# vressegu/sdeflow-light

Measured on AMD Instinct MI355X. Metric: score-matching train steps/sec (+ reverse-SDE sample steps/sec), higher is better.
Workload: dtype f32

## Files before the change

### sdeflow_light_amd/csrc/conv_kernels.hip

```cpp
#include "common.h"
#include <algorithm>
#include <type_traits>
#include <stdlib.h>

#define CONV_MAX_SRC 2

struct ConvGeom {
  int N, Hi, Wi, Ho, Wo;
  int KH, KW, strideH, padH, strideW, padW;
  int mode;
  int ups;
};

struct ConvArgs {
  ConvGeom g;
  const float* src[CONV_MAX_SRC];
  int C[CONV_MAX_SRC];
  int koff[CONV_MAX_SRC];
  int nsrc;
  const float* Wp;
  int Cout, CoutP, Ktot;
  const float* bias;
  const float* samp_bias;
  int n_bias, n_samp;
// ... 597 lines not shown
          if (dy > py || dx > px) continue;
          const int kh = py ? (dy ? 0 : 2) : 1, kw = px ? (dx ? 0 : 2) : 1;
          const float* wp = wl + (size_t)(kh * 3 + kw) * tap_stride + c0 + 16 * grp;
          f32x4 a[2];
#pragma unroll
          for (int c = 0; c < 2; ++c) a[c] = *reinterpret_cast<const f32x4*>(wp + c * co_stride);
#pragma unroll
          for (int r = 0; r < 4; ++r)
#pragma unroll
            for (int c = 0; c < 2; ++c)
#pragma unroll
              for (int pt = 0; pt < 2; ++pt) acc[cls][c][pt] = mfma16(a[c][r], b[pt][r], acc[cls][c][pt]);
        }
      }
    }
  }
  asm volatile("s_nop 15\n\ts_nop 7" ::: "memory");
  __builtin_amdgcn_sched_barrier(0);
#pragma unroll
  for (int c = 0; c < 2; ++c) {
    const int co = co0 + 16 * c + 4 * q;
    const f32x4 add = conv_addend(A, n, co, true);
    f32x4 cs = {0.f, 0.f, 0.f, 0.f}, css = cs;
#pragma unroll
    for (int pt = 0; pt < 2; ++pt) {
      const int yy = y0 + 2 * w + pt, xx = x0 + il;
      if (yy >= g.Hi || xx >= g.Wi) continue;
#pragma unroll
      for (int cls = 0; cls < 4; ++cls) {
        const size_t m = ((size_t)n * g.Ho + 2 * yy + (cls >> 1)) * g.Wo + 2 * xx + (cls & 1);
        conv_store_quad(A, A.out + m * A.Cout + co, acc[cls][c][pt] + add, true, co, cs, css);
      }
    }
  }
}

#define C1_LP 36
template <int PT, int KG, int EXTRA>
__global__ void __launch_bounds__(256) k_conv1x1(ConvArgs A, int P , long Mtot, int ct_per) {
  constexpr bool LDS_OUT = PT == 4;
  __shared__ __attribute__((aligned(16))) float c1_lds[4][LDS_OUT ? 16 * PT * C1_LP : 4];
  const int tid = threadIdx.x, w = tid >> 6, lane = tid & 63, il = lane & 15, q = lane >> 4;
  const long m0 = ((long)blockIdx.x * 4 + w) * (16 * PT);
  if (m0 >= Mtot) return;
  float* wl = c1_lds[w];
  const int n = __builtin_amdgcn_readfirstlane((int)(m0 / P));
  const int g0 = A.C[0] >> 4;
  const int ctot = A.C[0] + (A.nsrc > 1 ? A.C[1] : 0);
  f32x4 b[PT][KG];
#pragma unroll
  for (int pt = 0; pt < PT; ++pt) {
    const long m = m0 + 16 * pt + il;
#pragma unroll
    for (int g = 0; g < KG; ++g) {
      const bool second = g >= g0;
      const int c = (second ? 16 * (g - g0) : 16 * g) + 4 * q;
      const int C = second ? A.C[1] : A.C[0];
      b[pt][g] = *reinterpret_cast<const f32x4*>((second ? A.src[1] : A.src[0]) + (size_t)m * C + c);
    }
  }
  if (A.in_scale) {
#pragma unroll
    for (int g = 0; g < KG; ++g) {
      const bool second = g >= g0;
      const size_t o = (size_t)n * ctot + (second ? A.C[0] + 16 * (g - g0) : 16 * g) + 4 * q;
      const f32x4 ga = *reinterpret_cast<const f32x4*>(A.in_scale + o), gb = *reinterpret_cast<const f32x4*>(A.in_shift + o);
#pragma unroll
      for (int pt = 0; pt < PT; ++pt) {
        f32x4 v = b[pt][g] * ga + gb;
        if (A.in_act == 1) {
#pragma unroll
          for (int r = 0; r < 4; ++r) v[r] = v[r] * __builtin_amdgcn_rcpf(1.0f + __expf(-v[r]));
        }
        b[pt][g] = v;
      }
    }
  }
  const int ct0 = blockIdx.y * ct_per, ntile = min(A.Cout >> 4, ct0 + ct_per);
  const float* wrow = A.Wp + (size_t)il * A.Ktot + 4 * q;
  const size_t tile_stride = (size_t)16 * A.Ktot;
  constexpr int D = (KG % 4 == 0) ? 4 : 2;
  static_assert(KG % D == 0 && D <= KG, "ring slots must line up from one tile to the next");
  f32x4 an[D];
#pragma unroll
  for (int d = 0; d < D; ++d) an[d] = *reinterpret_cast<const f32x4*>(wrow + (size_t)ct0 * tile_stride + 16 * d);
  const bool has_b = A.bias && n < A.n_bias, has_s = A.samp_bias && n < A.n_samp;
  const float fb = has_b ? 1.f : 0.f, fs = has_s ? 1.f : 0.f;
  const float* bp = has_b ? A.bias + 4 * q : A.Wp;
  const float* sp = has_s ? A.samp_bias + (size_t)n * A.Cout + 4 * q : A.Wp;
  const int bstep = has_b ? 16 : 0, sstep = has_s ? 16 : 0;
  f32x4 add_n = *reinterpret_cast<const f32x4*>(bp + (size_t)ct0 * bstep) * fb + *reinterpret_cast<const f32x4*>(sp + (size_t)ct0 * sstep) * fs;
  const float* ex = EXTRA ? (A.residual ? A.residual : A.out) : nullptr;
  const size_t orow = (size_t)(m0 + il) * A.Cout + 4 * q;
  const size_t ptstep = (size_t)16 * A.Cout;
  f32x4 ex_n[EXTRA ? PT : 1];
  if (EXTRA) {
#pragma unroll
    for (int pt = 0; pt < PT; ++pt) ex_n[pt] = *reinterpret_cast<const f32x4*>(ex + orow + pt * ptstep + 16 * ct0);
  }
  for (int ct = ct0; ct < ntile; ++ct) {
    const int ctn = min(ct + 1, ntile - 1);
    f32x4 acc[PT];
#pragma unroll
    for (int pt = 0; pt < PT; ++pt) acc[pt] = f32x4{0, 0, 0, 0};
    const f32x4 add = add_n;
    f32x4 exv[EXTRA ? PT : 1];
    if (EXTRA) {
#pragma unroll
      for (int pt = 0; pt < PT; ++pt) exv[pt] = ex_n[pt];
    }
#pragma unroll
    for (int g = 0; g < KG; ++g) {
      const f32x4 a = an[g % D];
      const int ng = (g + D < KG) ? g + D : g + D - KG, nct = (g + D < KG) ? ct : ctn;
      an[g % D] = *reinterpret_cast<const f32x4*>(wrow + (size_t)nct * tile_stride + 16 * ng);
      if (g == 0) {
        add_n = *reinterpret_cast<const f32x4*>(bp + (size_t)ctn * bstep) * fb + *reinterpret_cast<const f32x4*>(sp + (size_t)ctn * sstep) * fs;
        if (EXTRA) {
#pragma unroll
          for (int pt = 0; pt < PT; ++pt) ex_n[pt] = *reinterpret_cast<const f32x4*>(ex + orow + pt * ptstep + 16 * ctn);
        }
      }
      __builtin_amdgcn_sched_barrier(0);
#pragma unroll
      for (int r = 0; r < 4; ++r)
#pragma unroll
        for (int pt = 0; pt < PT; ++pt) acc[pt] = mfma16(a[r], b[pt][g][r], acc[pt]);
    }
    f32x4 cs = {0.f, 0.f, 0.f, 0.f}, css = {0.f, 0.f, 0.f, 0.f};
    const int half = (ct - ct0) & 1;
    const bool paired = LDS_OUT && (half == 1 || ct + 1 < ntile);
#pragma unroll
    for (int pt = 0; pt < PT; ++pt) {
      f32x4 v = acc[pt] + add;
      if (EXTRA) v += exv[pt];
      if (paired) *reinterpret_cast<f32x4*>(wl + (16 * pt + il) * C1_LP + 16 * half + 4 * q) = v;
      else *reinterpret_cast<f32x4*>(A.out + orow + pt * ptstep + 16 * ct) = v;
      cs += v; css += v * v;
    }
    if (LDS_OUT && half == 1) {
      const size_t obase = (size_t)m0 * A.Cout + 16 * (ct - 1) + 4 * (lane & 7);
#pragma unroll
      for (int j = 0; j < 2 * PT; ++j) {
        const int px = 8 * j + (lane >> 3);
        const f32x4 v = *reinterpret_cast<const f32x4*>(wl + px * C1_LP + 4 * (lane & 7));
        *reinterpret_cast<f32x4*>(A.out + obase + (size_t)px * A.Cout) = v;
        if (j & 1) __builtin_amdgcn_sched_barrier(0);
      }
    }
    if (A.cstat) cstat_store(A, n, (int)((m0 % P) / (16 * PT)), 16 * ct + 4 * q, cs, css, il);
  }
}

constexpr int H18_HW = 18, H18_ITEMS = H18_HW * H18_HW * (CT_KC / 4), H18_NST = (H18_ITEMS + 255) / 256;
__device__ __forceinline__ void halo18_load(const ConvArgs& A, const ConvGeom& g, const float* src, int C, int up, int c0, size_t aff0, int n, int y0, int x0,
                                            int tid, f32x4 (&st)[H18_NST], unsigned& valid, f32x4& ga, f32x4& gb) {
  const float* base = src + (size_t)n * g.Hi * g.Wi * C;
  const int cq = c0 + 4 * (tid & 7);
  ga = f32x4{1.f, 1.f, 1.f, 1.f}; gb = f32x4{0.f, 0.f, 0.f, 0.f};
  if (A.in_scale && cq < C) {
    const size_t o = aff0 + cq;
    ga = *reinterpret_cast<const f32x4*>(A.in_scale + o);
    gb = *reinterpret_cast<const f32x4*>(A.in_shift + o);
  }
  valid = 0;
#pragma unroll
  for (int k = 0; k < H18_NST; ++k) {
    const int idx = tid + 256 * k;
    f32x4 v = {0, 0, 0, 0};
    if (idx < H18_ITEMS) {
      const int hp = idx >> 3, hy = hp / H18_HW, hx = hp - hy * H18_HW;
      const int iy = y0 + hy - 1, ix = x0 + hx - 1;
      const int c = c0 + 4 * (idx & 7);
      if (iy >= 0 && iy < (g.Hi << up) && ix >= 0 && ix < (g.Wi << up) && c < C) {
        v = *reinterpret_cast<const f32x4*>(base + ((size_t)(iy >> up) * g.Wi + (ix >> up)) * C + c);
        valid |= 1u << k;
      }
    }
    st[k] = v;
  }
}
__device__ __forceinline__ void halo18_store(const ConvArgs& A, float* buf, int tid, f32x4 (&st)[H18_NST], unsigned valid, f32x4 ga, f32x4 gb) {
  if (A.in_scale) {
#pragma unroll
    for (int k = 0; k < H18_NST; ++k) {
      if ((valid >> k) & 1u) {
        f32x4 v = st[k] * ga + gb;
        if (A.in_act == 1) {
#pragma unroll
          for (int r = 0; r < 4; ++r) v[r] = v[r] * __builtin_amdgcn_rcpf(1.0f + __expf(-v[r]));
        }
        st[k] = v;
      }
    }
  }
#pragma unroll
  for (int k = 0; k < H18_NST; ++k) {
    const int idx = tid + 256 * k;
    if (idx < H18_ITEMS) *reinterpret_cast<f32x4*>(buf + (idx >> 3) * CT_P + 4 * (idx & 7)) = st[k];
  }
}

__device__ __forceinline__ float wave64_sum_to_last(float v) {
  v = row16_sum(v);
  v += __builtin_bit_cast(float, __builtin_amdgcn_update_dpp(0, __builtin_bit_cast(int, v), 0x142, 0xA, 0xF, false));
  v += __builtin_bit_cast(float, __builtin_amdgcn_update_dpp(0, __builtin_bit_cast(int, v), 0x143, 0xC, 0xF, false));
  return v;
}

template <int CO>
__global__ void __launch_bounds__(256) k_conv3x3_cin_small(ConvArgs A, long Mtot) {
  const ConvGeom g = A.g;
  const int P = g.Ho * g.Wo, Cin = A.C[0];
  const long m = (long)blockIdx.x * 256 + threadIdx.x;
  const bool live = m < Mtot;
  const long mm = live ? m : Mtot - 1;
  const int n = (int)(mm / P), r = (int)(mm - (long)n * P), y = r / g.Wo, x = r - y * g.Wo;
  const float* src = A.src[0] + (size_t)n * g.Hi * g.Wi * Cin;
  float acc[CO];
#pragma unroll
  for (int co = 0; co < CO; ++co) acc[co] = 0.f;
#pragma unroll
  for (int tap = 0; tap < 9; ++tap) {
    const int iy = y + tap / 3 - 1, ix = x + tap % 3 - 1;
    const bool ok = iy >= 0 && iy < g.Hi && ix >= 0 && ix < g.Wi;
    const float* px = src + ((size_t)(ok ? iy : 0) * g.Wi + (ok ? ix : 0)) * Cin;
    const float* wt = A.Wp + (size_t)(g.mode ? 8 - tap : tap) * A.CoutP * A.Ktot;
    for (int c = 0; c < Cin; ++c) {
      const float xv = ok ? px[c] : 0.f;
#pragma unroll
      for (int co = 0; co < CO; ++co) acc[co] = __builtin_fmaf(xv, wt[(size_t)co * A.Ktot + c], acc[co]);
    }
  }
  const bool primal = n < A.n_bias && A.bias;
  float* op = A.out + (size_t)mm * CO;
#pragma unroll
  for (int c4 = 0; c4 < CO / 4; ++c4) {
    f32x4 v = {acc[4 * c4], acc[4 * c4 + 1], acc[4 * c4 + 2], acc[4 * c4 + 3]};
    if (primal) v += *reinterpret_cast<const f32x4*>(A.bias + 4 * c4);
    if (A.samp_bias && n < A.n_samp) v += *reinterpret_cast<const f32x4*>(A.samp_bias + (size_t)n * CO + 4 * c4);
    if (live) {
      if (A.accumulate) v += *reinterpret_cast<const f32x4*>(op + 4 * c4);
      if (A.residual) v += *reinterpret_cast<const f32x4*>(A.residual + (size_t)mm * CO + 4 * c4);
      *reinterpret_cast<f32x4*>(op + 4 * c4) = v;
    } else {
      v = f32x4{0.f, 0.f, 0.f, 0.f};
    }
#pragma unroll
    for (int k = 0; k < 4; ++k) acc[4 * c4 + k] = v[k];
  }
  if (A.cstat) {
    const int lane = threadIdx.x & 63;
    float* cp = A.cstat + (((size_t)n * A.cs_S + (r >> 6)) * 2) * CO;
#pragma unroll
    for (int co = 0; co < CO; ++co) {
      const float s = wave64_sum_to_last(acc[co]), ss = wave64_sum_to_last(acc[co] * acc[co]);
      if (lane == 63 && live) { cp[co] = s; cp[CO + co] = ss; }
    }
  }
}

template <int CO>
__global__ void __launch_bounds__(256) k_conv3x3_cout_small(ConvArgs A, int tiles_x, int tiles_y) {
  extern __shared__ __attribute__((aligned(16))) float cs_lds[];
  const ConvGeom g = A.g;
  const int tid = threadIdx.x;
  constexpr int HW = H18_HW;
  int n, y0, x0;
  tile_origin<16, 16>(blockIdx.x, tiles_x, tiles_y, n, y0, x0);
  f32x4 st[H18_NST], ga, gb;
  unsigned valid;
  halo18_load(A, g, A.src[0], 32, 0, 0, (size_t)n * 32, n, y0, x0, tid, st, valid, ga, gb);
  halo18_store(A, cs_lds, tid, st, valid, ga, gb);
  __syncthreads();
  const int py = tid >> 4, px = tid & 15;
  float acc[CO];
#pragma unroll
  for (int co = 0; co < CO; ++co) acc[co] = 0.f;
#pragma unroll
  for (int tap = 0; tap < 9; ++tap) {
    const float* xp = cs_lds + ((py + tap / 3) * HW + px + tap % 3) * CT_P;
    const float* wt = A.Wp + (size_t)tap * A.CoutP * A.Ktot;
#pragma unroll
    for (int q4 = 0; q4 < 8; ++q4) {
      const f32x4 xv = *reinterpret_cast<const f32x4*>(xp + 4 * q4);
#pragma unroll
      for (int co = 0; co < CO; ++co) {
        const float* w = wt + (size_t)co * A.Ktot + 4 * q4;
        acc[co] = __builtin_fmaf(xv[0], w[0], acc[co]); acc[co] = __builtin_fmaf(xv[1], w[1], acc[co]);
        acc[co] = __builtin_fmaf(xv[2], w[2], acc[co]); acc[co] = __builtin_fmaf(xv[3], w[3], acc[co]);
      }
    }
#pragma unroll
    for (int co = 0; co < CO; ++co) asm volatile("" : "+v"(acc[co]));
  }
  const int oy = y0 + py, ox = x0 + px;
  if (oy < g.Ho && ox < g.Wo) {
    const size_t m = ((size_t)n * g.Ho + oy) * g.Wo + ox;
    float* op = A.out + m * CO;
#pragma unroll
    for (int co = 0; co < CO; ++co) {
      float v = acc[co];
      if (n < A.n_bias && A.bias) v += A.bias[co];
      if (A.samp_bias && n < A.n_samp) v += A.samp_bias[(size_t)n * CO + co];
      if (A.accumulate) v += op[co];
      if (A.residual) v += A.residual[m * CO + co];
// ... 1410 lines not shown
    if (dual) zt = *reinterpret_cast<const f32x4*>(z + half + 4 * i);
    f32x4 hp, ht;
#pragma unroll
    for (int k = 0; k < 4; ++k) {
      float a0, a1, a2;
      if (ACT == 0) gelu012(zp[k], a0, a1, a2); else silu012(zp[k], a0, a1, a2);
      hp[k] = a0; ht[k] = a1 * zt[k];
    }
    *reinterpret_cast<f32x4*>(h + 4 * i) = hp;
    if (dual) *reinterpret_cast<f32x4*>(h + half + 4 * i) = ht;
  }
}
template <int ACT>
__global__ void k_act_dual_bwd(const float* __restrict__ z, float* __restrict__ g, int64_t half) {
  const int64_t nq = half >> 2;
  for (int64_t i = blockIdx.x * (int64_t)blockDim.x + threadIdx.x; i < nq; i += (int64_t)gridDim.x * blockDim.x) {
    const f32x4 zp = *reinterpret_cast<const f32x4*>(z + 4 * i), zt = *reinterpret_cast<const f32x4*>(z + half + 4 * i);
    f32x4 gp = *reinterpret_cast<const f32x4*>(g + 4 * i), gt = *reinterpret_cast<const f32x4*>(g + half + 4 * i);
#pragma unroll
    for (int k = 0; k < 4; ++k) {
      float a0, a1, a2;
      if (ACT == 0) gelu012(zp[k], a0, a1, a2); else silu012(zp[k], a0, a1, a2);
      const float np = gp[k] * a1 + gt[k] * (a2 * zt[k]);
      gt[k] = gt[k] * a1;
      gp[k] = np;
    }
    *reinterpret_cast<f32x4*>(g + 4 * i) = gp;
    *reinterpret_cast<f32x4*>(g + half + 4 * i) = gt;
  }
}

__device__ __forceinline__ void slot_reduce_block(long blk, const float* __restrict__ part, int nslots, long stride, long n_elem,
                                                  float* __restrict__ out, int C, int Ktot, int koff, int accumulate,
                                                  int rowsP, int rows, long n_elem2, float* __restrict__ out2) {
  __shared__ float red[8][32];
  const int el = threadIdx.x & 31, sl = threadIdx.x >> 5;
  const long nb1 = (n_elem + 31) / 32;
  if (blk >= nb1) {
    const long e2 = (blk - nb1) * 32 + el;
    const bool ok2 = e2 < n_elem2;
    float t2 = 0.f;
    if (ok2)
      for (int s = sl; s < nslots; s += 8) t2 += part[(size_t)s * stride + n_elem + e2];
    red[sl][el] = t2;
    __syncthreads();
    if (sl == 0 && ok2) {
      float r = red[0][el];
#pragma unroll
      for (int k = 1; k < 8; ++k) r += red[k][el];
      out2[e2] = accumulate ? out2[e2] + r : r;
    }
    return;
  }
  const long e = blk * 32 + el;
  const bool ok = e < n_elem && (rowsP == 0 || (int)((e / C) % rowsP) < rows);
  float t = 0.f;
  if (ok)
    for (int s = sl; s < nslots; s += 8) t += part[(size_t)s * stride + e];
  red[sl][el] = t;
  __syncthreads();
  if (sl == 0 && ok) {
    float r = red[0][el];
#pragma unroll
    for (int k = 1; k < 8; ++k) r += red[k][el];
    const long o = Ktot > 0 ? (e / C) * Ktot + koff + (e % C) : e;
    out[o] = accumulate ? out[o] + r : r;
  }
}
__global__ void __launch_bounds__(256) k_slot_reduce(const float* __restrict__ part, int nslots, long stride, long n_elem,
                                                      float* __restrict__ out, int C, int Ktot, int koff, int accumulate,
                                                      int rowsP, int rows, long n_elem2, float* __restrict__ out2) {
  slot_reduce_block((long)blockIdx.x, part, nslots, stride, n_elem, out, C, Ktot, koff, accumulate, rowsP, rows, n_elem2, out2);
}
__global__ void __launch_bounds__(256) k_slot_reduce_batched(const msgm_reduce_job_t* __restrict__ jobs, int n_jobs) {
  int lo = 0, hi = n_jobs - 1;
  const long blk = blockIdx.x;
  while (lo < hi) {
    const int mid = (lo + hi + 1) >> 1;
    if (jobs[mid].block_begin <= blk) lo = mid; else hi = mid - 1;
  }
  const msgm_reduce_job_t J = jobs[lo];
  slot_reduce_block(blk - J.block_begin, J.part, J.nslots, (long)J.stride, (long)J.n_elem, J.out, J.C, J.Ktot, J.koff, J.accumulate,
                    J.rowsP, J.rows, (long)J.n_elem2, J.out2);
}

__global__ void __launch_bounds__(256) k_colsum(const float* __restrict__ x, float* __restrict__ S, int P, int C, int chunk) {
  __shared__ float red[256];
  const int n = blockIdx.x;
  const float* xn = x + (size_t)n * P * C;
  const int p0 = blockIdx.y * chunk, p1 = min(p0 + chunk, P);
  for (int cb = 0; cb < C; cb += 256) {
    const int lanes_c = min(C - cb, 256);
    const int rows = 256 / lanes_c;
    const int c = threadIdx.x % lanes_c, pr = threadIdx.x / lanes_c;
    float s = 0.f;
    if (pr < rows)
      for (int p = p0 + pr; p < p1; p += rows) s += xn[(size_t)p * C + cb + c];
    red[threadIdx.x] = (pr < rows) ? s : 0.f;
    __syncthreads();
    if (pr == 0) {
      float t = 0.f;
      for (int r = 0; r < rows; ++r) t += red[r * lanes_c + c];
      S[((size_t)blockIdx.y * gridDim.x + n) * C + cb + c] = t;
    }
    __syncthreads();
  }
}

__global__ void k_add_row(float* __restrict__ x, const float* __restrict__ E, int N, int P, int C, int pos, float sgn) {
  const int64_t tot = (int64_t)N * C;
  for (int64_t e = blockIdx.x * (int64_t)blockDim.x + threadIdx.x; e < tot; e += (int64_t)gridDim.x * blockDim.x) {
    const int n = (int)(e / C), c = (int)(e - (int64_t)n * C);
    x[((size_t)n * P + pos) * C + c] += sgn * E[e];
  }
}

__global__ void k_gather_row(const float* __restrict__ x, float* __restrict__ out, int N, int P, int C, int pos) {
  const int64_t tot = (int64_t)N * C;
  for (int64_t e = blockIdx.x * (int64_t)blockDim.x + threadIdx.x; e < tot; e += (int64_t)gridDim.x * blockDim.x) {
    const int n = (int)(e / C), c = (int)(e - (int64_t)n * C);
    out[e] = x[((size_t)n * P + pos) * C + c];
  }
}

static int check_geom(const msgm_conv_geom_t* g) {
  if (!g || g->N <= 0 || g->Hi <= 0 || g->Wi <= 0 || g->Ho <= 0 || g->Wo <= 0 || g->KH <= 0 || g->KW <= 0 ||
      g->strideH <= 0 || g->padH < 0 || g->strideW <= 0 || g->padW < 0 || (g->mode != 0 && g->mode != 1) ||
      (g->ups != 0 && g->ups != 1))
    return MSGM_E_BADARG;
  if ((int64_t)g->N * g->Ho * g->Wo >= (1ll << 31) || (int64_t)g->N * g->Hi * g->Wi >= (1ll << 31)) return MSGM_E_UNSUPPORTED;
  return MSGM_OK;
}
static ConvGeom to_geom(const msgm_conv_geom_t* g) {
  return ConvGeom{g->N, g->Hi, g->Wi, g->Ho, g->Wo, g->KH, g->KW, g->strideH, g->padH, g->strideW, g->padW, g->mode, g->ups};
}

static bool conv_same(const msgm_conv_geom_t* g) {
  const int ups_sh = g->ups ? 1 : 0;
  return g->strideH == 1 && g->strideW == 1 && (g->Hi << ups_sh) == g->Ho && (g->Wi << ups_sh) == g->Wo &&
         (g->KH & 1) && (g->KW & 1) && g->KH <= 3 && g->KW <= 3 && g->padH == (g->KH - 1) / 2 && g->padW == (g->KW - 1) / 2;
}

static int conv_n_cu() {
  static const int n_cu = [] { int d = 0, n = 256; (void)hipGetDevice(&d); (void)hipDeviceGetAttribute(&n, hipDeviceAttributeMultiprocessorCount, d); return n > 0 ? n : 256; }();
  return n_cu;
}
template <auto K, int BYTES = 160 * 1024>
static void conv_raise_lds_limit() {
  static const int once = [] {
    (void)hipFuncSetAttribute(reinterpret_cast<const void*>(K), hipFuncAttributeMaxDynamicSharedMemorySize, BYTES);
    return 0;
  }();
  (void)once;
}

extern "C" {

static bool conv_tile_eligible(const msgm_conv_geom_t* geom, int32_t C0, bool has1, int32_t C1, int32_t CoutP) {
  const bool fast = (C0 % 16 == 0) && (!has1 || C1 % 16 == 0);
  return conv_same(geom) && (!geom->ups || geom->mode == 0) && fast && CoutP % 32 == 0 && (int64_t)geom->Ho * geom->Wo >= 64 &&
         (geom->Ho > 1 ? geom->KH == geom->KW : geom->KH == 1);
}

static bool conv_wino_eligible(const msgm_conv_geom_t* geom, int32_t C0, int32_t C1, int32_t CoutP, int cmul) {
  return geom->mode == 0 && geom->KH == 3 && geom->KW == 3 && conv_same(geom) && geom->Ho % 16 == 0 && geom->Wo % 16 == 0 &&
         C0 % cmul == 0 && C1 % cmul == 0 && CoutP % 32 == 0;
}

int msgm_conv_wino_supported(const msgm_conv_geom_t* geom, int32_t C0, int32_t C1, int32_t CoutP) {
  if (check_geom(geom)) return 0;
  return conv_wino_eligible(geom, C0, C1, CoutP, 16) ? 1 : 0;
}

static int conv_args(ConvArgs* A, const msgm_conv_geom_t* geom, const float* src0, int32_t C0, const float* src1, int32_t C1,
                     const void* W, int32_t Cout, int32_t CoutP, int32_t Ktot, const float* bias, const float* samp_bias,
                     int32_t n_bias, int32_t n_samp, float* out, int32_t accumulate, const msgm_conv_fuse_t* fuse,
                     bool padded_k) {
  int rc = check_geom(geom);
  if (rc) return rc;
  if (fuse && ((fuse->in_scale == nullptr) != (fuse->in_shift == nullptr) || (fuse->in_act != 0 && fuse->in_act != 1)))
    return MSGM_E_BADARG;
  if (!src0 || !W || !out || C0 <= 0 || Cout <= 0 || (src1 && C1 <= 0)) return MSGM_E_BADARG;
  const int k0 = padded_k ? ((C0 + 15) / 16) * 16 : C0, k1 = !src1 ? 0 : padded_k ? ((C1 + 15) / 16) * 16 : C1;
  if (Ktot != k0 + k1 || CoutP % 16 || CoutP < Cout) return MSGM_E_BADARG;
  *A = ConvArgs{};
  A->g = to_geom(geom);
  A->src[0] = src0; A->C[0] = C0; A->koff[0] = 0;
  A->src[1] = src1; A->C[1] = src1 ? C1 : 0; A->koff[1] = k0;
  A->nsrc = src1 ? 2 : 1;
  A->Wp = static_cast<const float*>(W); A->Cout = Cout; A->CoutP = CoutP; A->Ktot = Ktot;
  A->bias = bias; A->samp_bias = samp_bias; A->n_bias = n_bias; A->n_samp = n_samp; A->out = out; A->accumulate = accumulate;
  if (fuse) {
    A->residual = fuse->residual; A->in_scale = fuse->in_scale; A->in_shift = fuse->in_shift; A->in_act = fuse->in_act;
    for (int i = 0; i < 16; ++i) A->tapmask_in[i] = fuse->tapmask_in[i];
    for (int i = 0; i < 8; ++i) A->tapmask_out[i] = fuse->tapmask_out[i];
    A->cstat = fuse->chanstats;
  }
  return MSGM_OK;
}
static bool conv_has_masks(const ConvArgs& A) {
  unsigned m = 0;
  for (int i = 0; i < 16; ++i) m |= A.tapmask_in[i];
  for (int i = 0; i < 8; ++i) m |= A.tapmask_out[i];
  return m != 0;
}

int msgm_wino_pack_weights_batched(const msgm_pack_job_t* jobs, int32_t n_jobs, msgm_stream_t stream) {
  if (!jobs || n_jobs <= 0) return MSGM_E_BADARG;
  hipLaunchKernelGGL(k_wino_pack_batched, dim3(8, (unsigned)n_jobs), dim3(256), 0, S(stream), jobs);
  return msgm_check_launch();
}

static bool tile16_chanstats(ConvArgs& A) {
  if (!A.cstat) return true;
  A.cs_S = (A.g.Wo / 16) * (A.g.Ho / 16) * 4;
  return A.Cout % 4 == 0;
}

int msgm_conv_forward_wino(const msgm_conv_geom_t* geom, const float* src0, int32_t C0, const float* src1, int32_t C1,
                           const float* WpW, int32_t Cout, int32_t CoutP, int32_t Ktot, const float* bias,
                           const float* samp_bias, int32_t n_bias, int32_t n_samp, float* out, int32_t accumulate,
                           const msgm_conv_fuse_t* fuse, msgm_stream_t stream) {
  ConvArgs A;
  int rc = conv_args(&A, geom, src0, C0, src1, C1, WpW, Cout, CoutP, Ktot, bias, samp_bias, n_bias, n_samp, out, accumulate,
                     fuse, true);
  if (rc) return rc;
  if (!conv_wino_eligible(geom, C0, A.C[1], CoutP, 16) || !tile16_chanstats(A)) return MSGM_E_UNSUPPORTED;
  const int tiles_x = geom->Wo / 16, tiles_y = geom->Ho / 16;
  const int n_tiles = tiles_x * tiles_y * geom->N, gy = CoutP / 32;
  if (!A.in_scale) {
    const int64_t lim = (int64_t)1 << 31;
    if ((int64_t)geom->Hi * geom->Wi * std::max(C0, A.C[1]) * 4 >= lim || (int64_t)16 * CoutP * Ktot * 4 >= lim) return MSGM_E_UNSUPPORTED;
    conv_raise_lds_limit<&k_conv_wino_pipe, WP_LDS_BYTES>();
    const int items_per_xcd = gy * ((n_tiles + 7) / 8);
    const int wg_per_xcd = std::min(items_per_xcd, std::max(1, 2 * conv_n_cu() / 8));
    hipLaunchKernelGGL(k_conv_wino_pipe, dim3((unsigned)(8 * wg_per_xcd)), dim3(256), WP_LDS_BYTES, S(stream), A, tiles_x, tiles_y, n_tiles, gy);
    return msgm_check_launch();
  }
  const size_t lds = (size_t)18 * 18 * CT_P * sizeof(float);
  dim3 grid((unsigned)(8 * gy * ((n_tiles + 7) / 8)));
  constexpr int p32_min = 1024;
  if (!src1 && Ktot == 32 && CoutP == 32 && n_tiles >= p32_min) {
    conv_raise_lds_limit<&k_conv_wino_p32>();
    const size_t lds32 = ((size_t)2 * 16 * 2 * 256 + 2 * 18 * 18 * CT_P) * sizeof(float);
    hipLaunchKernelGGL(k_conv_wino_p32, dim3((unsigned)conv_n_cu()), dim3(256), lds32, S(stream), A, tiles_x, tiles_y, n_tiles);
    return msgm_check_launch();
  }
  if (Ktot < 64) {
    hipLaunchKernelGGL((k_conv_wino<2, false>), grid, dim3(256), lds, S(stream), A, tiles_x, tiles_y, n_tiles, gy);
    return msgm_check_launch();
  }
  conv_raise_lds_limit<&k_conv_wino<2, true>>();
  hipLaunchKernelGGL((k_conv_wino<2, true>), grid, dim3(256), lds + 2 * 4096 * sizeof(float), S(stream), A, tiles_x, tiles_y, n_tiles, gy);
  return msgm_check_launch();
}

__global__ void __launch_bounds__(256) k_b6_split(const float* __restrict__ Wp, __bf16* __restrict__ Wb, long n) {
  for (long e = (long)blockIdx.x * 256 + threadIdx.x; e < n; e += (long)gridDim.x * 256) {
    const float x = Wp[e];
    const __bf16 h = (__bf16)x;
    const float r1 = x - (float)h;
    const __bf16 m = (__bf16)r1;
    Wb[e] = h; Wb[n + e] = m; Wb[2 * n + e] = (__bf16)(r1 - (float)m);
  }
}

int msgm_conv_b6_supported(const msgm_conv_geom_t* geom, int32_t C0, int32_t C1, int32_t CoutP) {
  if (check_geom(geom)) return 0;
  return conv_wino_eligible(geom, C0, C1, CoutP, 32) ? 1 : 0;
}

int msgm_b6_split_weights(const float* Wp, void* Wb, int64_t n_elem, msgm_stream_t stream) {
  if (!Wp || !Wb || n_elem <= 0) return MSGM_E_BADARG;
  hipLaunchKernelGGL(k_b6_split, dim3((unsigned)grid_for(n_elem, 256, 2048)), dim3(256), 0, S(stream), Wp, static_cast<__bf16*>(Wb), (long)n_elem);
  return msgm_check_launch();
}

int msgm_conv_forward_b6(const msgm_conv_geom_t* geom, const float* src0, int32_t C0, const float* src1, int32_t C1,
                         const void* Wb, int32_t Cout, int32_t CoutP, int32_t Ktot, const float* bias,
                         const float* samp_bias, int32_t n_bias, int32_t n_samp, float* out, int32_t accumulate,
                         const msgm_conv_fuse_t* fuse, msgm_stream_t stream) {
  ConvArgs A;
  int rc = conv_args(&A, geom, src0, C0, src1, C1, Wb, Cout, CoutP, Ktot, bias, samp_bias, n_bias, n_samp, out, accumulate,
                     fuse, false);
  if (rc) return rc;
  if (!conv_wino_eligible(geom, C0, A.C[1], CoutP, 32) || conv_has_masks(A) || !tile16_chanstats(A)) return MSGM_E_UNSUPPORTED;
  const int nco = (CoutP % 64 == 0) ? 4 : 2;
  const int tiles_x = (geom->Wo + 15) / 16, tiles_y = (geom->Ho + 15) / 16;
  const int n_tiles = tiles_x * tiles_y * geom->N, gy = CoutP / (16 * nco);
  int per = (int)(((int64_t)n_tiles * gy) / (512 * 8));
  if (per > 4) per = 4;
  if (per < 1) per = 1;
  const int n_tgrp = (n_tiles + per - 1) / per;
  dim3 grid((unsigned)(8 * gy * ((n_tgrp + 7) / 8)));
  const size_t lds = (size_t)18 * 18 * 52 * sizeof(float);
  conv_raise_lds_limit<&k_conv_tile<16, 16, 4, 3, 4, false, true>>();
  conv_raise_lds_limit<&k_conv_tile<16, 16, 2, 3, 4, false, true>>();
  if (nco == 4) hipLaunchKernelGGL((k_conv_tile<16, 16, 4, 3, 4, false, true>), grid, dim3(256), lds, S(stream), A, 0, tiles_x, tiles_y, per, n_tiles, gy, n_tgrp);
  else hipLaunchKernelGGL((k_conv_tile<16, 16, 2, 3, 4, false, true>), grid, dim3(256), lds, S(stream), A, 0, tiles_x, tiles_y, per, n_tiles, gy, n_tgrp);
  return msgm_check_launch();
}

struct ConvRoute {
  int kind;
  int pt, kg;
  bool wide, two_d; int nco, TH, TW, tiles_x, tiles_y;
};
static bool conv_small_shape(const msgm_conv_geom_t* geom, bool has1, bool masks) {
  return conv_same(geom) && geom->KH == 3 && geom->KW == 3 && !geom->ups && geom->Ho > 1 && !has1 && !masks;
}
static bool conv_dgrad_s2_shape(const msgm_conv_geom_t* geom, int32_t C0, bool has1, int32_t Cout, int32_t CoutP, bool masks) {
  return geom->mode == 1 && geom->KH == 3 && geom->KW == 3 && geom->strideH == 2 && geom->strideW == 2 && geom->padH == 1 &&
         geom->padW == 1 && !geom->ups && geom->Ho == 2 * geom->Hi && geom->Wo == 2 * geom->Wi && !has1 && !masks &&
         C0 % 32 == 0 && Cout % 32 == 0 && CoutP == Cout;
}
static ConvRoute conv_route(const msgm_conv_geom_t* geom, int32_t C0, bool has1, int32_t C1, int32_t Cout, int32_t CoutP,
                            bool masks, bool both_extra = false , bool any_size = false) {
  ConvRoute r{};
  const int64_t Mtot = (int64_t)geom->N * geom->Ho * geom->Wo;
  if (conv_dgrad_s2_shape(geom, C0, has1, Cout, CoutP, masks)) { r.kind = 5; return r; }
  if (conv_small_shape(geom, has1, masks)) {
    if (C0 <= 4 && Cout == 32 && CoutP == 32) { r.kind = 3; return r; }
    if (C0 == 32 && Cout <= 4 && geom->mode == 0) { r.kind = 4; return r; }
  }
  const bool fast = (C0 % 16 == 0) && (!has1 || C1 % 16 == 0);
  const int Ktot = ((C0 + 15) / 16) * 16 + (has1 ? ((C1 + 15) / 16) * 16 : 0);
  const int kg = Ktot / 16;
  if (conv_same(geom) && geom->KH == 1 && geom->KW == 1 && !geom->ups && fast && !masks && (Mtot >= 4096 || any_size) &&
      (kg == 2 || kg == 4 || kg == 6 || kg == 8 || kg == 12 || kg == 16) && Cout % 16 == 0 && !both_extra) {
    const int pt = kg <= 4 ? 4 : (kg <= 8 ? 2 : (kg == 12 && (geom->Ho * geom->Wo) % 32 == 0 ? 2 : 1));
    if ((geom->Ho * geom->Wo) % (16 * pt) == 0) { r.kind = 1; r.kg = kg; r.pt = pt; return r; }
  }
  if (conv_tile_eligible(geom, C0, has1, C1, CoutP)) {
    r.kind = 2;
    r.two_d = geom->Ho > 1;
    r.nco = (CoutP % 64 == 0) ? 4 : 2;
    bool wide = geom->KW == 3 && (r.two_d ? (geom->Ho >= 16 && geom->Wo >= 16) : geom->Wo >= 256);
    if (wide) {
      const int64_t wtiles = (int64_t)geom->N * ((geom->Wo + (r.two_d ? 15 : 255)) / (r.two_d ? 16 : 256)) *
                             (r.two_d ? (geom->Ho + 15) / 16 : 1) * (CoutP / (16 * r.nco));
      if (wtiles < 512) wide = false;
    }
    r.wide = wide;
    r.TH = r.two_d ? (wide ? 16 : 8) : 1; r.TW = r.two_d ? 16 : (wide ? 256 : 128);
    r.tiles_x = (geom->Wo + r.TW - 1) / r.TW; r.tiles_y = (geom->Ho + r.TH - 1) / r.TH;
    if (!wide && r.nco == 4 && !masks && (int64_t)geom->N * r.tiles_x * r.tiles_y * (CoutP / 64) < 512) r.nco = 2;
    return r;
  }
  r.pt = (CoutP >= 64 && CoutP % 64 == 0) ? 2 : 4;
  return r;
}
static int conv_route_slots(const ConvRoute& r, const msgm_conv_geom_t* geom, int32_t Cout) {
  if (Cout % 4) return 0;
  if (r.kind == 1) { const int P = geom->Ho * geom->Wo; return P % (16 * r.pt) == 0 ? P / (16 * r.pt) : 0; }
  if (r.kind == 2) return r.tiles_x * r.tiles_y * 4;
  if (r.kind == 3) { const int P = geom->Ho * geom->Wo; return P % 64 == 0 ? P / 64 : 0; }
  if (r.kind == 4 || r.kind == 5) return 0;
  const int P = geom->Ho * geom->Wo, px = 16 * r.pt;
  return P % px == 0 ? P / px : 0;
}

int32_t msgm_conv_chanstats_slots(const msgm_conv_geom_t* geom, int32_t C0, int32_t C1, int32_t Cout, int32_t CoutP) {
  if (check_geom(geom) || C0 <= 0 || C1 < 0 || Cout <= 0 || CoutP < Cout || CoutP % 16) return 0;
  return conv_route_slots(conv_route(geom, C0, C1 > 0, C1, Cout, CoutP, false), geom, Cout);
}

static bool conv_in_transform_ok(const ConvRoute& r, const msgm_conv_geom_t* geom, int32_t C0, bool has1, int32_t C1, int32_t CoutP) {
  return r.kind == 4 || conv_tile_eligible(geom, C0, has1, C1, CoutP);
}

int msgm_conv_input_transform_supported(const msgm_conv_geom_t* geom, int32_t C0, int32_t C1, int32_t Cout, int32_t CoutP) {
  if (check_geom(geom)) return 0;
  return conv_in_transform_ok(conv_route(geom, C0, C1 > 0, C1, Cout, CoutP, false), geom, C0, C1 > 0, C1, CoutP) ? 1 : 0;
}

int msgm_conv_forward(const msgm_conv_geom_t* geom, const float* src0, int32_t C0, const float* src1, int32_t C1,
                      const float* Wp, int32_t Cout, int32_t CoutP, int32_t Ktot, const float* bias,
                      const float* samp_bias, int32_t n_bias, int32_t n_samp, float* out, int32_t accumulate,
                      msgm_stream_t stream) {
  return msgm_conv_forward_fused(geom, src0, C0, src1, C1, Wp, Cout, CoutP, Ktot, bias, samp_bias, n_bias, n_samp, out,
                                 accumulate, nullptr, stream);
}

int msgm_conv_forward_fused(const msgm_conv_geom_t* geom, const float* src0, int32_t C0, const float* src1, int32_t C1,
                            const float* Wp, int32_t Cout, int32_t CoutP, int32_t Ktot, const float* bias,
                            const float* samp_bias, int32_t n_bias, int32_t n_samp, float* out, int32_t accumulate,
                            const msgm_conv_fuse_t* fuse, msgm_stream_t stream) {
  ConvArgs A;
  int rc = conv_args(&A, geom, src0, C0, src1, C1, Wp, Cout, CoutP, Ktot, bias, samp_bias, n_bias, n_samp, out, accumulate,
                     fuse, true);
  if (rc) return rc;
  const bool masks = conv_has_masks(A);
  const bool both_extra = accumulate && A.residual;
  msgm_conv_geom_t lin = *geom;
  const bool as_pixels = geom->Hi == 1 && geom->Wi == 1 && geom->Ho == 1 && geom->Wo == 1 && geom->KH == 1 && geom->KW == 1 &&
                         geom->N >= 32 && !samp_bias && (!bias || n_bias >= geom->N) && !A.in_scale && !A.cstat;
  if (as_pixels) {
    lin.Wi = lin.Wo = geom->N; lin.N = 1; lin.mode = 0;
    const ConvRoute rl = conv_route(&lin, C0, src1 != nullptr, C1, Cout, CoutP, masks, both_extra, true);
    if (rl.kind == 1) { geom = &lin; A.g = to_geom(geom); A.n_bias = bias ? 1 : 0; A.n_samp = 0; }
  }
  const ConvRoute rt = conv_route(geom, C0, src1 != nullptr, C1, Cout, CoutP, masks, both_extra, geom == &lin);
  if (A.in_scale && !conv_in_transform_ok(rt, geom, C0, src1 != nullptr, C1, CoutP)) return MSGM_E_UNSUPPORTED;
  const int64_t Mtot = (int64_t)geom->N * geom->Ho * geom->Wo;
  const bool fast = (C0 % 16 == 0) && (!src1 || C1 % 16 == 0);
  if (A.cstat) {
    A.cs_S = masks ? 0 : conv_route_slots(rt, geom, Cout);
    if (A.cs_S == 0 || A.cs_S != msgm_conv_chanstats_slots(geom, C0, src1 ? C1 : 0, Cout, CoutP)) return MSGM_E_UNSUPPORTED;
  }
  if (rt.kind == 3) {
    hipLaunchKernelGGL((k_conv3x3_cin_small<32>), dim3((unsigned)((Mtot + 255) / 256)), dim3(256), 0, S(stream), A, (long)Mtot);
    return msgm_check_launch();
  }
  if (rt.kind == 4) {
    const int tiles_x = (geom->Wo + 15) / 16, tiles_y = (geom->Ho + 15) / 16;
    const dim3 grid((unsigned)(tiles_x * tiles_y * geom->N));
    const size_t lds = (size_t)18 * 18 * CT_P * sizeof(float);
    switch (Cout) {
      case 1: hipLaunchKernelGGL((k_conv3x3_cout_small<1>), grid, dim3(256), lds, S(stream), A, tiles_x, tiles_y); break;
      case 2: hipLaunchKernelGGL((k_conv3x3_cout_small<2>), grid, dim3(256), lds, S(stream), A, tiles_x, tiles_y); break;
      case 3: hipLaunchKernelGGL((k_conv3x3_cout_small<3>), grid, dim3(256), lds, S(stream), A, tiles_x, tiles_y); break;
      default: hipLaunchKernelGGL((k_conv3x3_cout_small<4>), grid, dim3(256), lds, S(stream), A, tiles_x, tiles_y); break;
    }
    return msgm_check_launch();
  }
  if (rt.kind == 5) {
    const int tiles_x = (geom->Wi + DS_TW - 1) / DS_TW, tiles_y = (geom->Hi + DS_TH - 1) / DS_TH, n_cob = Cout / 32;
    const int64_t wgs = (int64_t)geom->N * tiles_x * tiles_y * n_cob;
    if (wgs >= (1ll << 31)) return MSGM_E_UNSUPPORTED;
    hipLaunchKernelGGL(k_dgrad_s2, dim3((unsigned)wgs), dim3(256), 0, S(stream), A, tiles_x, tiles_y, n_cob);
    return msgm_check_launch();
  }
  if (rt.kind == 1) {
    const int P = geom->Ho * geom->Wo;
    const int ntile = (Cout + 15) / 16;
    const long wgs = (Mtot + 64 * rt.pt - 1) / (64 * rt.pt);
    int split = wgs >= 768 ? 1 : (int)((768 + wgs - 1) / wgs);
    if (split > ntile) split = ntile;
    const int ct_per = (ntile + split - 1) / split, gy = (ntile + ct_per - 1) / ct_per;
    const bool extra = accumulate || A.residual;
#define C1_LAUNCH(PT_, KG_)                                                                                          \
  do {                                                                                                               \
    if (extra) hipLaunchKernelGGL((k_conv1x1<PT_, KG_, 1>), dim3((unsigned)wgs, (unsigned)gy), dim3(256), 0, S(stream), A, P, (long)Mtot, ct_per); \
    else hipLaunchKernelGGL((k_conv1x1<PT_, KG_, 0>), dim3((unsigned)wgs, (unsigned)gy), dim3(256), 0, S(stream), A, P, (long)Mtot, ct_per); \
  } while (0)
    switch (rt.kg) {
      case 2: C1_LAUNCH(4, 2); break;
      case 4: C1_LAUNCH(4, 4); break;
      case 6: C1_LAUNCH(2, 6); break;
      case 8: C1_LAUNCH(2, 8); break;
      case 12: if (rt.pt == 2) C1_LAUNCH(2, 12); else C1_LAUNCH(1, 12); break;
      default: C1_LAUNCH(1, 16); break;
    }
#undef C1_LAUNCH
    return msgm_check_launch();
  }
  if (rt.kind == 2) {
    const bool two_d = rt.two_d, wide = rt.wide;
    const int nco = rt.nco, TH = rt.TH, TW = rt.TW, tiles_x = rt.tiles_x, tiles_y = rt.tiles_y;
    const int halo = (TH + geom->KH - 1) * (TW + geom->KW - 1);
    const size_t lds = (size_t)(wide ? 1 : 2) * halo * CT_P * sizeof(float);
    const int n_tiles = tiles_x * tiles_y * geom->N, gy = CoutP / (16 * nco);
    constexpr int max_per = 4, rounds = 8;
    int per = (int)(((int64_t)n_tiles * gy) / (768 * rounds));
    if (per > max_per) per = max_per;
    if (per < 1) per = 1;
    const int n_tgrp = (n_tiles + per - 1) / per;
    dim3 grid((unsigned)(8 * gy * ((n_tgrp + 7) / 8)));
    const int flip = geom->mode;
#define CT_LAUNCH(TH_, TW_, NCO_, KS_, PT_, DB_) \
  hipLaunchKernelGGL((k_conv_tile<TH_, TW_, NCO_, KS_, PT_, DB_>), grid, dim3(256), lds, S(stream), A, flip, tiles_x, tiles_y, per, n_tiles, gy, n_tgrp)
    const bool k3 = geom->KW == 3;
    if (two_d) {
      if (wide) { if (nco == 4) CT_LAUNCH(16, 16, 4, 3, 4, false); else CT_LAUNCH(16, 16, 2, 3, 4, false); }
      else if (nco == 4) { if (k3) CT_LAUNCH(8, 16, 4, 3, 2, true); else CT_LAUNCH(8, 16, 4, 1, 2, true); }
      else { if (k3) CT_LAUNCH(8, 16, 2, 3, 2, true); else CT_LAUNCH(8, 16, 2, 1, 2, true); }
    } else {
      if (wide) { if (nco == 4) CT_LAUNCH(1, 256, 4, 3, 4, false); else CT_LAUNCH(1, 256, 2, 3, 4, false); }
      else if (nco == 4) { if (k3) CT_LAUNCH(1, 128, 4, 3, 2, true); else CT_LAUNCH(1, 128, 4, 1, 2, true); }
      else { if (k3) CT_LAUNCH(1, 128, 2, 3, 2, true); else CT_LAUNCH(1, 128, 2, 1, 2, true); }
    }
#undef CT_LAUNCH
    return msgm_check_launch();
  }
  if (CoutP >= 64 && CoutP % 64 == 0) {
    dim3 grid((unsigned)((Mtot + 4 * 32 - 1) / (4 * 32)), (unsigned)(CoutP / 64));
    if (fast) hipLaunchKernelGGL((k_conv_gemm<4, 2, true>), grid, dim3(256), 0, S(stream), A);
    else hipLaunchKernelGGL((k_conv_gemm<4, 2, false>), grid, dim3(256), 0, S(stream), A);
  } else if (CoutP % 32 == 0) {
    dim3 grid((unsigned)((Mtot + 4 * 64 - 1) / (4 * 64)), (unsigned)(CoutP / 32));
    if (fast) hipLaunchKernelGGL((k_conv_gemm<2, 4, true>), grid, dim3(256), 0, S(stream), A);
    else hipLaunchKernelGGL((k_conv_gemm<2, 4, false>), grid, dim3(256), 0, S(stream), A);
  } else {
    dim3 grid((unsigned)((Mtot + 4 * 64 - 1) / (4 * 64)), (unsigned)(CoutP / 16));
    if (fast) hipLaunchKernelGGL((k_conv_gemm<1, 4, true>), grid, dim3(256), 0, S(stream), A);
    else hipLaunchKernelGGL((k_conv_gemm<1, 4, false>), grid, dim3(256), 0, S(stream), A);
  }
  return msgm_check_launch();
}

struct WgradPlan { bool tile; int wgs, per, tiles_x, tiles_y, n_tiles, yblocks; int64_t nchunks, chunk; int64_t bias_slots, bias_chunk;
                   bool one; int mt, nt, wm, px; int64_t n_tiles1; bool wino;
                   int th, tw; size_t lds; };
static void wgrad1x1_shape(int C, int Cout, int* mt, int* nt, int* wm) {
  *mt = 0; *nt = 0; *wm = 4;
  if (C != 32 && C != 64 && C != 128 && C != 256) return;
  if (Cout == 32 && C <= 128) { *mt = 1; *nt = C / 32; *wm = 2; return; }
  if (Cout % 64) return;
  *nt = C / 16;
  if (C == 256) { *mt = 1; return; }
  *mt = Cout % 192 == 0 ? 3 : (Cout % 128 == 0 ? 2 : 1);
}
static WgradPlan wgrad_plan(const msgm_conv_geom_t* geom, int C, int Cout, int n_bias, bool wino) {
  WgradPlan p{};
  const int64_t Mtot = (int64_t)geom->N * geom->Ho * geom->Wo;
  const int taps = geom->KH * geom->KW;
  const bool same = geom->mode == 0 && conv_same(geom);
  if (taps == 1 && same && !geom->ups && geom->padH == 0 && geom->padW == 0 && ((int64_t)n_bias * geom->Ho * geom->Wo) % 16 == 0) {
    wgrad1x1_shape(C, Cout, &p.mt, &p.nt, &p.wm);
    if (p.mt) {
      p.one = true;
      const int COB = 16 * p.mt * p.wm, Wd = COB + C;
      p.px = w1_px(Wd);
      p.lds = (size_t)2 * p.px * (Wd + 4) * sizeof(float);
      p.yblocks = Cout / COB;
      p.n_tiles1 = (Mtot + p.px - 1) / p.px;
      int wgs = 512 / p.yblocks;
      int64_t per = (p.n_tiles1 + wgs - 1) / wgs;
      int per_min = COB * C / 4096;
      per_min = per_min < 2 ? 2 : (per_min > 8 ? 8 : per_min);
      if (per < per_min) per = p.n_tiles1 < per_min ? p.n_tiles1 : per_min;
      p.per = (int)per;
      p.wgs = (int)((p.n_tiles1 + per - 1) / per);
      return p;
    }
  }
  const bool aligned = C % 4 == 0 && Cout % 4 == 0;
  p.tile = same && (aligned || (taps == 9 && geom->Ho > 1)) && (int64_t)geom->Ho * geom->Wo >= 64 &&
           (taps == 1 || taps == 3 || (taps == 9 && geom->Ho > 1)) && (geom->Ho > 1 || geom->KH == 1);
  if (p.tile) {
    const bool two_d = geom->Ho > 1;
    p.th = two_d ? 8 : 1; p.tw = two_d ? 16 : 128;
    p.tiles_x = (geom->Wo + p.tw - 1) / p.tw; p.tiles_y = (geom->Ho + p.th - 1) / p.th;
    p.n_tiles = p.tiles_x * p.tiles_y * geom->N;
    p.yblocks = ((Cout + 31) / 32) * ((C + 31) / 32);
    p.wino = wino && two_d && taps == 9 && aligned;
    const int kw = wt_kw(p.th, taps), ip = wt_in_pitch(wt_halo(p.th, p.tw, taps / kw, kw));
    p.lds = sizeof(float) * (p.wino ? 2 * wt_buf_floats(WW_IP) : (taps == 9 && aligned ? 1 : wt_tile_bufs(taps)) * wt_buf_floats(ip));
    const int wg_target = p.wino ? 256 * 2 : 768;
    int wgs = wg_target / p.yblocks;
    if (wgs < 1) wgs = 1;
    int per = (p.n_tiles + wgs - 1) / wgs;
    constexpr int min_per = 8;
    if (per < min_per) per = p.n_tiles < min_per ? p.n_tiles : min_per;
    if (per < 1) per = 1;
    p.per = per;
    p.wgs = (p.n_tiles + per - 1) / per;
    return p;
  }
  const int coblocks = (Cout + 31) / 32, cblocks = (C + 63) / 64;
  int64_t nchunks = 2048 / (int64_t)(coblocks * cblocks * taps);
  if (nchunks < 1) nchunks = 1;
  int64_t chunk = (Mtot + nchunks - 1) / nchunks;
  if (chunk < 256) chunk = 256;
  chunk = ((chunk + 15) / 16) * 16;
  p.nchunks = (Mtot + chunk - 1) / chunk;
  p.chunk = chunk;
  p.yblocks = coblocks * cblocks;
  if (n_bias > 0) {
    const int64_t Pb = (int64_t)n_bias * geom->Ho * geom->Wo;
    int64_t cch = (Pb + 1023) / 1024;
    if (cch < 64) cch = 64;
    if (cch > Pb) cch = Pb;
    p.bias_chunk = cch;
    p.bias_slots = (Pb + cch - 1) / cch;
  }
  return p;
}

static int wgrad_impl(const msgm_conv_geom_t* geom, const float* gy, const float* src, int32_t C, int32_t koff,
                      float* dWp, int32_t Cout, int32_t CoutP, int32_t Ktot, float* dbias, int32_t n_bias,
                      const uint16_t* tapmask_c32, const uint16_t* tapmask_co32, float* ws, size_t ws_bytes,
                      int32_t wino, msgm_stream_t stream, msgm_reduce_job_t* jobs_out = nullptr, int32_t* n_jobs_out = nullptr);

size_t msgm_conv_wgrad_workspace(const msgm_conv_geom_t* geom, int32_t C, int32_t Cout, int32_t CoutP, int32_t n_bias, int32_t wino) {
  if (check_geom(geom) || C <= 0 || Cout <= 0 || CoutP < Cout) return 0;
  const WgradPlan p = wgrad_plan(geom, C, Cout, n_bias, wino != 0);
  const size_t stride = (size_t)geom->KH * geom->KW * CoutP * C + CoutP;
  const size_t slots = (p.tile || p.one) ? (size_t)p.wgs : (size_t)p.nchunks;
  return (slots * stride + (size_t)p.bias_slots * Cout) * sizeof(float);
}

int msgm_conv_wgrad_det(const msgm_conv_geom_t* geom, const float* gy, const float* src, int32_t C, int32_t koff,
// ... 237 lines not shown
```

Measured before the change: 10.66.

## Add LDS-resident-weight persistent 1x1 conv kernel with occupancy-sized grid

```diff
diff --git a/sdeflow_light_amd/csrc/conv_kernels.hip b/sdeflow_light_amd/csrc/conv_kernels.hip
--- a/sdeflow_light_amd/csrc/conv_kernels.hip
+++ b/sdeflow_light_amd/csrc/conv_kernels.hip
@@ -773,6 +773,126 @@
   }
 }
 
+template <int PT, int KG, int EXTRA, int NW>
+__global__ void __launch_bounds__(64 * NW) k_conv1x1_lds(ConvArgs A, int P , long Mtot) {
+  constexpr bool LDS_OUT = PT == 4;
+  constexpr int KQ = 4 * KG;
+  extern __shared__ __attribute__((aligned(16))) float c1s_lds[];
+  const int tid = threadIdx.x, w = tid >> 6, lane = tid & 63, il = lane & 15, q = lane >> 4;
+  const int ntile = A.Cout >> 4;
+  f32x4* wimg = reinterpret_cast<f32x4*>(c1s_lds);
+  {
+    const int items = ntile * 16 * KQ;
+    for (int i0 = tid; i0 < items; i0 += 4 * 64 * NW) {
+      f32x4 v[4];
+      int dst[4];
+#pragma unroll
+      for (int u = 0; u < 4; ++u) {
+        const int i = min(i0 + u * 64 * NW, items - 64 + lane);
+        const int blk = i >> 6, ko = blk % (KQ / 8), row = (blk / (KQ / 8)) * 8 + (i & 7), kq = ko * 8 + ((i >> 3) & 7);
+        v[u] = *reinterpret_cast<const f32x4*>(A.Wp + (size_t)row * A.Ktot + 4 * kq);
+        dst[u] = ((row >> 4) * KQ + kq) * 16 + (row & 15);
+      }
+#pragma unroll
+      for (int u = 0; u < 4; ++u)
+        if (i0 + u * 64 * NW < items) wimg[dst[u]] = v[u];
+    }
+  }
+  __syncthreads();
+  float* wl = c1s_lds + (size_t)ntile * 16 * KQ * 4 + (LDS_OUT ? w * (16 * PT * C1_LP) : 0);
+  const f32x4* wa = wimg + q * 16 + il;
+  const int g0 = A.C[0] >> 4;
+  const float* ex = EXTRA ? (A.residual ? A.residual : A.out) : nullptr;
+  const size_t ptstep = (size_t)16 * A.Cout;
+  constexpr long WG_PX = (long)NW * 16 * PT;
+  auto load_b = [&](auto& bb, long mm0) {
+#pragma unroll
+    for (int pt = 0; pt < PT; ++pt) {
+      const long m = mm0 + 16 * pt + il;
+#pragma unroll
+      for (int g = 0; g < KG; ++g) {
+        const bool second = g >= g0;
+        const int c = (second ? 16 * (g - g0) : 16 * g) + 4 * q;
+        const int C = second ? A.C[1] : A.C[0];
+        bb[pt][g] = *reinterpret_cast<const f32x4*>((second ? A.src[1] : A.src[0]) + (size_t)m * C + c);
+      }
+    }
+  };
+  const long mstep = (long)gridDim.x * WG_PX;
+  long m0 = (long)blockIdx.x * WG_PX + w * (16 * PT);
+  for (; m0 < Mtot; m0 += mstep) {
+    const int n = __builtin_amdgcn_readfirstlane((int)(m0 / P));
+    f32x4 b[PT][KG];
+    load_b(b, m0);
+    constexpr int D = PT == 4 ? 1 : (PT == 2 ? 2 : 4);
+    static_assert(KG % D == 0 && D <= KG, "ring slots must line up from one tile to the next");
+    f32x4 an[D];
+#pragma unroll
+    for (int d = 0; d < D; ++d) an[d] = wa[(4 * d) * 16];
+    const bool has_b = A.bias && n < A.n_bias, has_s = A.samp_bias && n < A.n_samp;
+    const float fb = has_b ? 1.f : 0.f, fs = has_s ? 1.f : 0.f;
+    const float* bp = has_b ? A.bias + 4 * q : A.Wp;
+    const float* sp = has_s ? A.samp_bias + (size_t)n * A.Cout + 4 * q : A.Wp;
+    const int bstep = has_b ? 16 : 0, sstep = has_s ? 16 : 0;
+    f32x4 add_n = *reinterpret_cast<const f32x4*>(bp) * fb + *reinterpret_cast<const f32x4*>(sp) * fs;
+    const size_t orow = (size_t)(m0 + il) * A.Cout + 4 * q;
+    f32x4 ex_n[EXTRA ? PT : 1];
+    if (EXTRA) {
+#pragma unroll
+      for (int pt = 0; pt < PT; ++pt) ex_n[pt] = *reinterpret_cast<const f32x4*>(ex + orow + pt * ptstep);
+    }
+    for (int ct = 0; ct < ntile; ++ct) {
+      const int ctn = min(ct + 1, ntile - 1);
+      f32x4 acc[PT];
+#pragma unroll
+      for (int pt = 0; pt < PT; ++pt) acc[pt] = f32x4{0, 0, 0, 0};
+      const f32x4 add = add_n;
+      f32x4 exv[EXTRA ? PT : 1];
+      if (EXTRA) {
+#pragma unroll
+        for (int pt = 0; pt < PT; ++pt) exv[pt] = ex_n[pt];
+      }
+#pragma unroll
+      for (int g = 0; g < KG; ++g) {
+        const f32x4 a = an[g % D];
+        const int ng = (g + D < KG) ? g + D : g + D - KG, nct = (g + D < KG) ? ct : ctn;
+        an[g % D] = wa[(nct * KQ + 4 * ng) * 16];
+        if (g == 0) {
+          add_n = *reinterpret_cast<const f32x4*>(bp + (size_t)ctn * bstep) * fb + *reinterpret_cast<const f32x4*>(sp + (size_t)ctn * sstep) * fs;
+          if (EXTRA) {
+#pragma unroll
+            for (int pt = 0; pt < PT; ++pt) ex_n[pt] = *reinterpret_cast<const f32x4*>(ex + orow + pt * ptstep + 16 * ctn);
+          }
+        }
+        __builtin_amdgcn_sched_barrier(0);
+#pragma unroll
+        for (int r = 0; r < 4; ++r)
+#pragma unroll
+          for (int pt = 0; pt < PT; ++pt) acc[pt] = mfma16(a[r], b[pt][g][r], acc[pt]);
+      }
+      const int half = ct & 1;
+      const bool paired = LDS_OUT && (half == 1 || ct + 1 < ntile);
+#pragma unroll
+      for (int pt = 0; pt < PT; ++pt) {
+        f32x4 v = acc[pt] + add;
+        if (EXTRA) v += exv[pt];
+        if (paired) *reinterpret_cast<f32x4*>(wl + (16 * pt + il) * C1_LP + 16 * half + 4 * q) = v;
+        else *reinterpret_cast<f32x4*>(A.out + orow + pt * ptstep + 16 * ct) = v;
+      }
+      if (LDS_OUT && half == 1) {
+        const size_t obase = (size_t)m0 * A.Cout + 16 * (ct - 1) + 4 * (lane & 7);
+#pragma unroll
+        for (int j = 0; j < 2 * PT; ++j) {
+          const int px = 8 * j + (lane >> 3);
+          const f32x4 v = *reinterpret_cast<const f32x4*>(wl + px * C1_LP + 4 * (lane & 7));
+          *reinterpret_cast<f32x4*>(A.out + obase + (size_t)px * A.Cout) = v;
+          if (j & 1) __builtin_amdgcn_sched_barrier(0);
+        }
+      }
+    }
+  }
+}
+
 constexpr int H18_HW = 18, H18_ITEMS = H18_HW * H18_HW * (CT_KC / 4), H18_NST = (H18_ITEMS + 255) / 256;
 __device__ __forceinline__ void halo18_load(const ConvArgs& A, const ConvGeom& g, const float* src, int C, int up, int c0, size_t aff0, int n, int y0, int x0,
                                             int tid, f32x4 (&st)[H18_NST], unsigned& valid, f32x4& ga, f32x4& gb) {
@@ -2489,6 +2609,29 @@
     return 0;
   }();
   (void)once;
+}
+
+template <int PT, int KG, int EXTRA, int NW>
+static void conv1x1_lds_launch(const ConvArgs& A, int P, int64_t Mtot, size_t lds, hipStream_t stream) {
+  conv_raise_lds_limit<&k_conv1x1_lds<PT, KG, EXTRA, NW>>();
+  static size_t seen_lds = 0;
+  static int per_cu = 1;
+  if (seen_lds != lds) {
+    int n = 0;
+    if (hipOccupancyMaxActiveBlocksPerMultiprocessor(&n, k_conv1x1_lds<PT, KG, EXTRA, NW>, 64 * NW, lds) != hipSuccess || n < 1) n = 1;
+    per_cu = n; seen_lds = lds;
+  }
+  const int64_t ntw = (Mtot + NW * 16 * PT - 1) / (NW * 16 * PT), cap = (int64_t)per_cu * conv_n_cu();
+  const int64_t rounds = (ntw + cap - 1) / cap, gx = (ntw + rounds - 1) / rounds;
+  hipLaunchKernelGGL((k_conv1x1_lds<PT, KG, EXTRA, NW>), dim3((unsigned)gx), dim3(64 * NW), lds, stream, A, P, (long)Mtot);
+}
+template <int PT, int KG>
+static void conv1x1_lds_dispatch(int nw, bool extra, const ConvArgs& A, int P, int64_t Mtot, size_t lds, hipStream_t stream) {
+  if (nw == 8) {
+    if (extra) conv1x1_lds_launch<PT, KG, 1, 8>(A, P, Mtot, lds, stream); else conv1x1_lds_launch<PT, KG, 0, 8>(A, P, Mtot, lds, stream);
+  } else {
+    if (extra) conv1x1_lds_launch<PT, KG, 1, 4>(A, P, Mtot, lds, stream); else conv1x1_lds_launch<PT, KG, 0, 4>(A, P, Mtot, lds, stream);
+  }
 }
 
 extern "C" {
@@ -2641,6 +2784,7 @@
 struct ConvRoute {
   int kind;
   int pt, kg;
+  int nw;
   bool wide, two_d; int nco, TH, TW, tiles_x, tiles_y;
 };
 static bool conv_small_shape(const msgm_conv_geom_t* geom, bool has1, bool masks) {
@@ -2651,6 +2795,22 @@
          geom->padW == 1 && !geom->ups && geom->Ho == 2 * geom->Hi && geom->Wo == 2 * geom->Wi && !has1 && !masks &&
          C0 % 32 == 0 && Cout % 32 == 0 && CoutP == Cout;
 }
+constexpr int C1S_LDS_MAX = 160 * 1024;
+static size_t conv1x1_lds_bytes(int kg, int pt, int Cout, int nw) {
+  return (size_t)Cout * 16 * kg * 4 + (pt == 4 ? (size_t)nw * 16 * pt * C1_LP * 4 : 0);
+}
+static int conv1x1_lds_waves(int kg, int pt, int Cout, int64_t Mtot) {
+  if (Mtot / (64 * pt) < 768 || kg < 4 || (size_t)Cout * 16 * kg * 4 > 128 * 1024) return 0;
+  int best = 0, best_waves = 0;
+  for (int nw : {4, 8}) {
+    const size_t lds = conv1x1_lds_bytes(kg, pt, Cout, nw);
+    if (lds > (size_t)C1S_LDS_MAX) break;
+    const int waves = std::min(12, (int)(C1S_LDS_MAX / lds) * nw);
+    if (waves > best_waves) { best = nw; best_waves = waves; }
+  }
+  return best;
+}
+
 static ConvRoute conv_route(const msgm_conv_geom_t* geom, int32_t C0, bool has1, int32_t C1, int32_t Cout, int32_t CoutP,
                             bool masks, bool both_extra = false , bool any_size = false) {
   ConvRoute r{};
@@ -2666,7 +2826,11 @@
   if (conv_same(geom) && geom->KH == 1 && geom->KW == 1 && !geom->ups && fast && !masks && (Mtot >= 4096 || any_size) &&
       (kg == 2 || kg == 4 || kg == 6 || kg == 8 || kg == 12 || kg == 16) && Cout % 16 == 0 && !both_extra) {
     const int pt = kg <= 4 ? 4 : (kg <= 8 ? 2 : (kg == 12 && (geom->Ho * geom->Wo) % 32 == 0 ? 2 : 1));
-    if ((geom->Ho * geom->Wo) % (16 * pt) == 0) { r.kind = 1; r.kg = kg; r.pt = pt; return r; }
+    if ((geom->Ho * geom->Wo) % (16 * pt) == 0) {
+      r.kind = 1; r.kg = kg; r.pt = pt;
+      r.nw = conv1x1_lds_waves(kg, pt, Cout, Mtot);
+      return r;
+    }
   }
   if (conv_tile_eligible(geom, C0, has1, C1, CoutP)) {
     r.kind = 2;
@@ -2776,6 +2940,18 @@
     if (split > ntile) split = ntile;
     const int ct_per = (ntile + split - 1) / split, gy = (ntile + ct_per - 1) / ct_per;
     const bool extra = accumulate || A.residual;
+    if (rt.nw && !A.in_scale && !A.cstat) {
+      const size_t lds = conv1x1_lds_bytes(rt.kg, rt.pt, Cout, rt.nw);
+      switch (rt.kg) {
+        case 4: conv1x1_lds_dispatch<4, 4>(rt.nw, extra, A, P, Mtot, lds, S(stream)); break;
+        case 6: conv1x1_lds_dispatch<2, 6>(rt.nw, extra, A, P, Mtot, lds, S(stream)); break;
+        case 8: conv1x1_lds_dispatch<2, 8>(rt.nw, extra, A, P, Mtot, lds, S(stream)); break;
+        case 12: if (rt.pt == 2) conv1x1_lds_dispatch<2, 12>(rt.nw, extra, A, P, Mtot, lds, S(stream));
+                 else conv1x1_lds_dispatch<1, 12>(rt.nw, extra, A, P, Mtot, lds, S(stream)); break;
+        default: conv1x1_lds_dispatch<1, 16>(rt.nw, extra, A, P, Mtot, lds, S(stream)); break;
+      }
+      return msgm_check_launch();
+    }
 #define C1_LAUNCH(PT_, KG_)                                                                                          \
   do {                                                                                                               \
     if (extra) hipLaunchKernelGGL((k_conv1x1<PT_, KG_, 1>), dim3((unsigned)wgs, (unsigned)gy), dim3(256), 0, S(stream), A, P, (long)Mtot, ct_per); \
```

After: 10.72, median of 6. Within noise of the previous version (+0.6%).
